# astomodynamics/cddp-cpp

Hardware: AMD Instinct MI355X
Metric: trajectories_per_sec (higher is better)
Workload: dtype f64

## Files before the change

cddp-cpp_amd/csrc/capi.hip:

```cpp
#include <algorithm>
#include <chrono>
#include <cmath>
#include <cstdarg>
#include <cstddef>
#include <cstdio>
#include <cstdlib>
#include <cstring>
#include <string>
#include <vector>
#include <map>

#include "launch.hpp"
#include "plant.hpp"
#include "io_kernels.hpp"
#include "sens_kernels.hpp"
#include "score_kernels.hpp"
#include "mppi_kernels.hpp"

static int ladder_strictly_decreasing(const double *a, int n) {
  for (int i = 1; i < n; ++i) if (!(a[i] < a[i - 1])) return 0;
  return n > 0 ? 1 : 0;
}

using namespace cddp_dev;
// ... 153 lines not shown
  bool initialized = false;
  bool has_state = false;
  bool initial_dirty = false;
  bool ms_cache_started = false;
  size_t bytes = 0;
  int timing_detail = CDDP_HIP_TIMING_ROLLOUT;
  std::vector<hipEvent_t> ev_pool;
  hipEvent_t ev_begin = nullptr, ev_end = nullptr, ev_poll = nullptr, ev_poll2 = nullptr;
  double *d_head = nullptr, *h_head = nullptr; size_t head_cap = 0;
  int *h_poll = nullptr;
  std::map<unsigned long long, hipGraphExec_t> graphs;
  bool shadow_bufs = false;
  int cs_epoch = 0;
  unsigned long long *h_ls = nullptr;
  long long ls_counts[3] = {0, 0, 0};
  int n_redo = 0;
  bool last_shadow = false;
  bool ever_solved = false;
  int *h_bad = nullptr;
  bool has_plan = false;
  double *d_xnext = nullptr;
  double *d_log_u = nullptr, *d_log_x = nullptr; int32_t *d_log_it = nullptr, *d_log_st = nullptr; int log_steps = 0;
};

namespace {

template <class T>
int dalloc(Inner *h, T **p, size_t n) {
  if (n == 0) n = 1;
  void *q = nullptr;
// ... 424 lines not shown
    DA(d.STt, (size_t)d.n_alphas * 8 * Bp); DA(d.YTt, (size_t)d.n_alphas * 8 * Bp); DA(d.GTt, (size_t)d.n_alphas * 8 * Bp);
    DA(d.LamTt, (size_t)d.n_alphas * 16 * Bp);
    if (P.pT > 0) {
      const bool te_coop = h->ks->te_rec_size > 0 && P.mT == 0 && P.pT + 1 <= h->ks->te_group && P.pT <= P.nx;
      const size_t nv = te_coop ? 16 : (size_t)(P.pT + 1);
      DA(d.te_k, nv * N * nu * Bp); DA(d.te_p, nv * (N + 1) * nx * Bp);
      if (te_coop) {
        DA(d.te_cst, (size_t)N * h->ks->te_rec_size * Bp); DA(d.te_cnt, Bp);
        if (!d.dX) DA(d.dX, (size_t)N * nx * Bp);
        if (!d.ys) DA(d.ys, (size_t)N * (m > 0 ? m : 1) * Bp);
      }
    }
  }
  DA(d.n_active, 1);
  DA(d.win_hist, CDDP_HIP_MAX_ALPHAS + 1);
  DA(h->d_launched, ls_words(Bp / 64));
  DA(h->dP, 1);
  DA(h->d_Xinit, d.planeX); DA(h->d_Uinit, d.planeU);
  if (problem->x_ref_traj) {
    DA(h->d_xref_traj, (size_t)(N + 1) * nx);
    hipMemcpyAsync(h->d_xref_traj, problem->x_ref_traj, sizeof(double) * (N + 1) * nx, hipMemcpyHostToDevice, h->stream);
    d.xref_traj = h->d_xref_traj;
  }
#undef DA
  hipMemcpyAsync(h->dP, &h->P, sizeof(ProblemDev), hipMemcpyHostToDevice, h->stream);
  d.P = h->dP;
  d.launched = h->d_launched;
  resolve_route(h);
  if (shadow_layout(h) && knob.costate != Knobs::kCostateSync && !knob.fail_costate && !knob.graph) {
#define DA(ptr, n) do { int rc_ = dalloc(h, &(ptr), (size_t)(n)); if (rc_) { in_destroy(h); return rc_; } } while (0)
    DA(d.Vx2, (size_t)(N + 1) * nx * Bp); DA(d.Vxx2, (size_t)(N + 1) * nx * nx * Bp);
// ... 278 lines not shown
  return 0;
}

struct SolveRun {
  Inner *h = nullptr;
  bool want_stats = false;
  int conc = 1;
  int detail = -1;
  std::vector<int> ev_slot;
  size_t ev_used = 0;
  int launches = 0, outer = 0, it = 0, max_it = 0, na = 0;
  bool two_stage_marks = false, first_rule = true, pinned = false, one_stage = true, done = false, cpu_time_hit = false, use_graph = false;
  int k1 = 1, k_cap = 1, k_cap2 = 1;
  bool shadow = false, force_sync = false, pre_has_state = false, redo_needed = false;
  bool inkernel = false;
  int poll_us = kLsPollUs;
  int stamp0 = 0;
  long waves_all = 0, per_alpha_waves = 1, two_stage_max_waves = 768;
  std::vector<int> hist_now, hist_prev;
  static constexpr int kPollWords = CDDP_HIP_MAX_ALPHAS + 2;
  hipEvent_t poll_evs[2] = {nullptr, nullptr};
  int win_enq = 0, win_dig = 0, win_it[2] = {0, 0};
  int outstanding() const { return win_enq - win_dig; }
  bool ran_ahead = false;
  int post_poll(hipStream_t s) {
    const int slot = win_enq & 1;
    HIPCHK(hipMemcpyAsync(h->h_poll + slot * kPollWords, h->d.n_active, sizeof(int), hipMemcpyDeviceToHost, s));
    HIPCHK(hipMemcpyAsync(h->h_poll + slot * kPollWords + 1, h->d.win_hist, sizeof(int) * (na + 1), hipMemcpyDeviceToHost, s));
    HIPCHK(hipEventRecord(poll_evs[slot], s));
    win_it[slot] = it;
    ++win_enq;
    return 0;
  }
  std::chrono::steady_clock::time_point wall0;
  hipEvent_t fwd_wait = nullptr, fwd_done = nullptr;

  void mark(int point) {
    if (detail < 0) return;
    const bool want = detail == CDDP_HIP_TIMING_ALL ||
                      (detail == CDDP_HIP_TIMING_ROLLOUT && (point == 1 || point == 2 || (two_stage_marks && (point == 3 || point == 4)))) ||
                      (detail == CDDP_HIP_TIMING_SWEEP && (point == 0 || point == 1));
    if (!want) return;
    if (ev_used == h->ev_pool.size()) {
      hipEvent_t e;
      if ((h->knob->event_fence ? hipEventCreate(&e) : hipEventCreateWithFlags(&e, hipEventDisableSystemFence)) != hipSuccess) return;
      h->ev_pool.push_back(e);
    }
    const size_t slot = (size_t)6 * (size_t)(outer - 1) + (size_t)point;
    if (ev_slot.size() <= slot) ev_slot.resize(slot + 1, -1);
    hipEventRecord(h->ev_pool[ev_used], h->stream);
    ev_slot[slot] = (int)ev_used++;
  }

  void adapt_ladder(int window_iters) {
    if (pinned) return;
    long total = 0;
    std::vector<long> hd(na + 1);
    for (int a = 0; a <= na; ++a) { hd[a] = (long)hist_now[a] - (long)hist_prev[a]; total += hd[a]; }
    hist_prev = hist_now;
    if (total <= 0) return;
    const long allow = std::max(1L, (long)window_iters / 4);
    int kq = na;
    long tail = hd[na];
    for (int k = na - 1; k >= 1; --k) {
      tail += hd[k];
      if (tail <= allow) kq = k; else break;
    }
    if (kq >= na - 1) {
      if (waves_all <= 2048) { one_stage = true; }
      else { one_stage = false; k1 = k_cap2; }
    } else {
      one_stage = false; k1 = std::max(1, std::min(kq + h->knob->ls_margin, k_cap));
      if (waves_all <= 2048 && (long)k1 * per_alpha_waves > two_stage_max_waves) one_stage = true;
      const long small_cap = (h->P.solver == CDDP_HIP_SOLVER_LOGDDP || h->P.solver == CDDP_HIP_SOLVER_MSIPDDP) ? 2048 : 1024;
      if (waves_all <= small_cap && h->P.nx <= 8 && h->knob->ls_small_frac * k1 > na) one_stage = true;
    }
    if (h->knob->debug_ladder) {
      std::fprintf(stderr, "[ladder] it=%d total=%ld kq=%d -> %s k1=%d hist:", outer, total, kq, one_stage ? "one" : "two", k1);
      for (int a = 0; a <= na; ++a) std::fprintf(stderr, " %ld", hd[a]);
      std::fprintf(stderr, "\n");
    }
  }

  int begin(Inner *h_, bool stats_, int conc_) {
    h = h_; want_stats = stats_; conc = std::max(1, conc_);
    const ProblemDev &P = h->P;
    const DevBuf &d = h->d;
    hipStream_t s = h->stream;
    const KernelSet *ks = h->ks;
    max_it = P.opt.max_iterations;
    first_rule = (P.ls_rule == CDDP_HIP_LS_FIRST_SUCCESS);
    na = d.n_alphas;
    use_graph = h->knob->graph;
    if (use_graph && conc > 1) {
// ... 3 lines not shown
    detail = (want_stats && !use_graph) ? h->timing_detail : -1;
    if (!h->ev_begin) { HIPCHK(hipEventCreate(&h->ev_begin)); HIPCHK(hipEventCreate(&h->ev_end)); }
    if (!h->ev_poll) { HIPCHK(hipEventCreateWithFlags(&h->ev_poll, hipEventDisableTiming)); HIPCHK(hipEventCreateWithFlags(&h->ev_poll2, hipEventDisableTiming)); }
    poll_evs[0] = h->ev_poll; poll_evs[1] = h->ev_poll2;
    win_enq = win_dig = 0; ran_ahead = false;
    if (!h->h_poll) HIPCHK(hipHostMalloc((void **)&h->h_poll, sizeof(int) * 2 * kPollWords));
    HIPCHK(hipMemsetAsync(h->d_launched, 0, sizeof(unsigned long long) * kLsGran, s));
    HIPCHK(hipEventRecord(h->ev_begin, s));
    pre_has_state = h->has_state;
    shadow = !force_sync && shadow_eligible(h, conc) && max_it > 0;
    redo_needed = false;
    inkernel = shadow && P.ls_rule == CDDP_HIP_LS_FIRST_SUCCESS && h->knob->ls_inkernel &&
               (h->route.rollout == Route::kPair || h->route.rollout == Route::kTwoConsumers);
    poll_us = h->knob->ls_poll_us >= 0 ? h->knob->ls_poll_us : kLsPollUs;
    h->ls_counts[0] = h->ls_counts[1] = h->ls_counts[2] = 0;
    if (inkernel && !h->h_ls) HIPCHK(hipHostMalloc((void **)&h->h_ls, sizeof(unsigned long long) * kLsGran));
    h->last_shadow = shadow; h->ever_solved = true;
    if (shadow) HIPCHK(hipMemsetAsync(h->d.cs_bad, 0, sizeof(int), s));
    stamp0 = h->cs_epoch;
    { int rc = run_initialize(h); if (rc) return rc; }
    launches = 1; outer = 0; it = 0; done = false;
    *h->h_poll = d.B;
    waves_all = (long)conc * (long)((d.B + 63) / 64) * na * (((P.solver == CDDP_HIP_SOLVER_IPDDP && (ks->cst_size > 0 || (d.te_cst && P.m > 0))) || P.solver == CDDP_HIP_SOLVER_MSIPDDP || P.solver == CDDP_HIP_SOLVER_LOGDDP) ? 2 : 1);
    const bool force_two = h->knob->ls_stages == '2', force_one = h->knob->ls_stages == '1';
    const long per_alpha = std::max(1L, waves_all / std::max(1, na));
    per_alpha_waves = per_alpha;
    two_stage_max_waves = h->knob->ls_two_max_waves;
    k_cap = (int)std::max(1L, std::min((long)na - 1, 1024 / per_alpha));
    k_cap2 = (int)std::max(1L, std::min((long)na - 1, 2048 / per_alpha));
    const int k_forced = h->knob->ls_first;
    pinned = !first_rule || na == 1 || force_one || force_two || (k_forced >= 1 && k_forced < na);
    one_stage = !first_rule || na == 1 || force_one || (waves_all <= 2048 && !force_two);
    k1 = force_two ? 1 : k_cap2;
    if (k_forced >= 1 && k_forced < na && !force_one && first_rule) { one_stage = false; k1 = k_forced; }
    hist_now.assign(na + 1, 0); hist_prev.assign(na + 1, 0);
    HIPCHK(hipMemsetAsync(d.win_hist, 0, sizeof(int) * (CDDP_HIP_MAX_ALPHAS + 1), s));
    wall0 = std::chrono::steady_clock::now();
    if (max_it <= 0) { ks->update(d, h->route, 2, 0, 1, 1, s); ++launches; done = true; }
    return 0;
  }

  void enqueue_iteration(int last) {
    const ProblemDev &P = h->P;
    if (shadow) {
      DevBuf &hd = h->d;
      hd.Vx_prev = hd.Vx; hd.Vxx_prev = hd.Vxx;
      std::swap(hd.Vx, hd.Vx2); std::swap(hd.Vxx, hd.Vxx2);
      hd.cs_vsel ^= 1;
    }
    DevBuf dsh = h->d;
    if (shadow) {
      h->cs_epoch += 2;
      dsh.cs_mode = 1; dsh.cs_stamp = h->cs_epoch + 1; dsh.cs_want = dsh.cs_stamp - 2;
      dsh.cs_fail_stamp = h->knob->fail_shadow > 0 ? stamp0 + 2 * h->knob->fail_shadow + 1 : 0;
    }
    const DevBuf &d = dsh;
    hipStream_t s = h->stream;
    const KernelSet *ks = h->ks;
    const Route &r = h->route;
    hipStream_t sf = h->cu.fwd ? h->cu.fwd : s;
    auto to_fwd = [&](int k) { if (sf != s) { order_check(hipEventRecord(h->cu.ev[k], s)); order_check(hipStreamWaitEvent(sf, h->cu.ev[k], 0)); } };
    auto from_fwd = [&](int k) { if (sf != s) { order_check(hipEventRecord(h->cu.ev[k], sf)); order_check(hipStreamWaitEvent(s, h->cu.ev[k], 0)); } };
    const bool split = !one_stage && inkernel;
    two_stage_marks = !one_stage && !split;
    mark(0);
    ks->derivs(d, r, 0, s);
    tl_sweep_hop = h->cu.sweep ? &h->cu.hop : nullptr;
    if (shadow && outer > 1) { dsh.cs_extra = ks->shadow_extra(d, r); ks->backward(dsh, r, P.solver, 0, 1, s); dsh.cs_extra = 0; }
    else ks->backward(d, r, P.solver, 0, 1, s);
    tl_sweep_hop = nullptr;
    mark(1);
    to_fwd(0);
    if (fwd_wait) hipStreamWaitEvent(sf, fwd_wait, 0);
    if (one_stage || split) {
      ks->forward(d, r, P.solver, 0, na, PH_FWD1, 0, first_rule ? 1 : 0, sf, split ? k1 : 0, poll_us);
      if (fwd_done) hipEventRecord(fwd_done, sf);
      from_fwd(1);
      mark(2);
      if (!shadow) ks->costate(d, r, P.solver, 0, na, PH_FWD1, 0, first_rule ? 1 : 2, s);
      ks->update(d, r, 1, na, last, 1, s);
      mark(3);
      launches += shadow ? 3 : 4;
    } else {
      ks->forward(d, r, P.solver, 0, k1, PH_FWD1, 0, 1, sf, 0, 0);
      from_fwd(1);
      mark(2);
      if (!shadow) ks->costate(d, r, P.solver, 0, k1, PH_FWD1, 0, 1, s);
      if (shadow) {
        DevBuf d1 = dsh;
        d1.cs_stamp = h->cs_epoch;
        ks->update(d1, r, 1, k1, last, 0, s);
        d1.cs_want = d1.cs_stamp; d1.Vx_prev = d1.Vx; d1.Vxx_prev = d1.Vxx;
        ks->shadow_flush(d1, nullptr, s);
      } else
      ks->update(d, r, 1, k1, last, 0, s);
      mark(3);
      to_fwd(2);
      ks->forward(d, r, P.solver, k1, na - k1, PH_FWD2, 0, 1, sf, 0, 0);
      if (fwd_done) hipEventRecord(fwd_done, sf);
      from_fwd(3);
      mark(4);
      if (!shadow) ks->costate(d, r, P.solver, k1, na - k1, PH_FWD2, 0, 1, s);
      ks->update(d, r, 2, na, last, 1, s);
      mark(5);
      launches += shadow ? 5 : 6;
    }
  }
  bool polled_iteration(int i) const { return i % h->knob->poll_every == 0 || i == max_it || (i <= 2 && !pinned); }

  int advance_graph() {
    const hipStream_t s = h->stream;
    int w = 0;
    while (it + w < max_it) { ++w; if (polled_iteration(it + w)) break; }
    if (w == 0) { done = true; return 0; }
    const int last = (it + w == max_it) ? 1 : 0;
    const unsigned long long key = ((unsigned long long)(one_stage ? 0 : k1) << 16) | ((unsigned long long)w << 4) | (unsigned long long)last;
    auto f = h->graphs.find(key);
    if (f == h->graphs.end()) {
      hipGraph_t g = nullptr; hipGraphExec_t ge = nullptr;
      const int launches0 = launches;
      HIPCHK(hipStreamBeginCapture(s, hipStreamCaptureModeThreadLocal));
      for (int j = 1; j <= w; ++j) enqueue_iteration((j == w) ? last : 0);
      HIPCHK(hipStreamEndCapture(s, &g));
// ... 62 lines not shown
      df.cs_mode = 1; df.cs_want = h->cs_epoch > stamp0 ? h->cs_epoch + 1 : 0; df.Vx_prev = df.Vx; df.Vxx_prev = df.Vxx;
      df.cs_fail_stamp = h->knob->fail_shadow > 0 ? stamp0 + 2 * h->knob->fail_shadow + 1 : 0;
      h->ks->shadow_flush(df, &dm, s);
      launches += df.cs_want > 0 ? 2 : 1;
      HIPCHK(hipMemsetD32Async((hipDeviceptr_t)d.cs_vbuf, d.cs_vsel, (size_t)d.Bp, s));
      HIPCHK(hipMemcpyAsync(h->h_bad, d.cs_bad, sizeof(int), hipMemcpyDeviceToHost, s));
    }
    return 0;
  }

  int finish(cddp_hip_stats *stats) {
    const DevBuf &d = h->d;
    hipStream_t s = h->stream;
    HIPCHK(hipEventRecord(h->ev_end, s));
    if (inkernel) HIPCHK(hipMemcpyAsync(h->h_ls, h->d_launched, sizeof(unsigned long long) * kLsGran, hipMemcpyDeviceToHost, s));
    HIPCHK(hipStreamSynchronize(s));
    HIPCHK(hipGetLastError());
    if (inkernel) { h->ls_counts[0] = (long long)h->h_ls[kLsRan]; h->ls_counts[1] = (long long)h->h_ls[kLsRet]; h->ls_counts[2] = (long long)h->h_ls[kLsGiveUp]; }
    if (shadow && *h->h_bad != 0) { redo_needed = true; return 0; }
    if (tl_order_error != hipSuccess) {
      const hipError_t oe = tl_order_error; tl_order_error = hipSuccess;
      return fail(-10, "stream ordering (event record / wait) failed during the solve: %s", hipGetErrorString(oe));
    }
    if (!stats) return 0;
    std::memset(stats, 0, sizeof(*stats));
    float ms = 0;
    hipEventElapsedTime(&ms, h->ev_begin, h->ev_end);
    stats->solve_ms = ms;
    auto span = [&](size_t it0, int pa, int pb) -> double {
      const size_t ia = it0 * 6 + (size_t)pa, ib = it0 * 6 + (size_t)pb;
      if (ib >= ev_slot.size() || ev_slot[ia] < 0 || ev_slot[ib] < 0) return 0.0;
      float v = 0;
// ... 427 lines not shown
  if (!h) return -1;
  for (Inner *q : h->g) if (!(q->ever_solved ? q->last_shadow : shadow_eligible(q, std::max(1, std::min(h->conc, (int)h->g.size()))))) return 0;
  return 1;
}
int cddp_hip_costate_redos(cddp_hip_handle *h) {
  if (!h) return -1;
  int n = 0;
  for (Inner *q : h->g) n += q->n_redo;
  return n;
}
int cddp_hip_ls_stage_counts(cddp_hip_handle *h, long long *counts) {
  if (!h || !counts) return -1;
  counts[0] = counts[1] = counts[2] = 0;
  for (Inner *q : h->g) for (int i = 0; i < 3; ++i) counts[i] += q->ls_counts[i];
  return 0;
}
int cddp_hip_concurrency(cddp_hip_handle *h) { return h ? std::max(1, std::min(h->conc, (int)h->g.size())) : -1; }

int cddp_hip_set_timing_detail(cddp_hip_handle *h, int detail) {
  if (!h) return fail(-1, "null handle");
  for (Inner *q : h->g) { int rc = in_set_timing_detail(q, detail); if (rc) return rc; }
  return 0;
}

int cddp_hip_set_stream(cddp_hip_handle *h, void *hip_stream) {
  if (!h) return fail(-1, "null handle");
  h->user_stream = (hipStream_t)hip_stream; h->have_user_stream = true;
  if (h->g.size() == 1) return in_set_stream(h->g[0], hip_stream);
  return 0;
}
// ... 987 lines not shown
```

cddp-cpp_amd/csrc/dev_types.hpp:

```cpp
#pragma once
#include <stdint.h>
#include <stddef.h>
#include "../../include/cddp_hip.h"

namespace cddp_dev {

constexpr int kMaxCons = 4;
constexpr int kMaxTerms = 2;
constexpr int kPool = 1024;
constexpr int kFilterCap = 8;
constexpr int kHistCols = 9;

enum Phase : int { PH_ACTIVE = 0, PH_FWD1 = 1, PH_FWD2 = 2, PH_DONE = 3 };

struct ConDev {
  int kind, dim, dual_dim, offset;
  int off_lower, off_upper, off_center, off_A, off_b;
  int _pad;
  double scale, radius;
};

struct TermDev {
  int kind, dim, offset;
  int off_target, off_A, off_b;
// ... 9 lines not shown
  ConDev cons[kMaxCons];
  TermDev terms[kMaxTerms];
  int off_Qdt, off_Rdt, off_Qf, off_xref;
  double alphas[CDDP_HIP_MAX_ALPHAS];
  double pool[kPool];
};

constexpr int kLS = 64;

constexpr int kSinkDoubles = 1024 * 64;

constexpr int kLsRan = 1, kLsRet = 2, kLsGiveUp = 3, kLsGran = 8;
constexpr unsigned kLsTag = 0x4c533231u;
constexpr size_t ls_words(int NB) { return (size_t)kLsGran + (size_t)NB * CDDP_HIP_MAX_ALPHAS * 2; }
constexpr int kLsPollUs = 10000;

struct DevBuf {
  int B, Bp, N, n_slots, n_alphas, hist_batch, hist_cap, NB;
  int fail_costate_mask;
  const ProblemDev *P;
  const double *xref_traj;
  double *X, *U, *S, *Y, *G, *Lam;
  size_t planeX, planeU, planeM;
  double *A, *Bm, *K, *k, *Vx, *Vxx, *ks, *ky, *Ks, *Ky;
  double *ST, *YT, *GT, *dST, *dYT, *LamT, *dLamT;
  double *STt, *YTt, *GTt, *LamTt;
  double *te_k, *te_p;
  double *te_cst;
  int *te_cnt;
  double *cost, *merit, *inf_pr, *inf_du, *inf_comp, *step_norm, *alpha_pr, *alpha_du, *reg, *mu;
// ... 49 lines not shown
```

cddp-cpp_amd/csrc/kernels.hpp:

```cpp
#pragma once
#include "dev_constraints.hpp"
#include "dev_boxqp.hpp"
#include "dev_models.hpp"
#include "dev_terminal.hpp"

namespace cddp_dev {

#define GI(t, E, e) (((((size_t)(t)) * (size_t)d.NB + (size_t)(b >> 6)) * (E) + (e)) * 64 + (size_t)(b & 63))
#define PIPELINE_FENCE() asm volatile("" ::: "memory")
#define RING_FENCE() asm volatile("s_waitcnt lgkmcnt(0)" ::: "memory")
#define GT(t, E, e) (d.t4 ? ((((size_t)(t) * (size_t)d.NB * 16 + (size_t)(b >> 2)) * (size_t)(E) + (size_t)(e)) * 4 + (size_t)(b & 3)) : GI(t, E, e))
#define G4(t, E, e) ((((size_t)(t) * (size_t)d.NB * 16 + (size_t)(b >> 2)) * (size_t)(E) + (size_t)(e)) * 4 + (size_t)(b & 3))
#define TSTRIDE (d.t4 ? (size_t)4 : (size_t)kLS)

constexpr double kSlackInteriorOffset = 1e-4;
constexpr double kEpsSlack = 1e-10;
constexpr double kMaxBarrierRatio = 1e6;

DEV double clip_pos(double num, double den) { return dclamp(num / den, 0.0, kMaxBarrierRatio); }
DEV double clip_sgn(double num, double den) { return dclamp(num / den, -kMaxBarrierRatio, kMaxBarrierRatio); }

template <int N> DEV void ld(const double *base, size_t stride, double *out) {
#pragma unroll
  for (int i = 0; i < N; ++i) out[i] = base[(size_t)i * stride];
// ... 1453 lines not shown
  const size_t ti = (size_t)a * d.Bp + b;
  const int slot = (a < cur) ? a : a + 1;
  const double a_pr = d.t_apr[ti];
  if ((d.fail_costate_mask >> a) & 1) return false;
  for (int t = 0; t <= d.N; ++t) {
    double xo[NX], lo[NX], vx[NX], xn[NX], lam[NX], vt[NX * (NX + 1) / 2];
    ld<NX>(d.X + (size_t)cur * d.planeX + GI(t, NX, 0), kLS, xo);
    ld<NX>(d.Lam + (size_t)cur * d.planeX + GI(t, NX, 0), kLS, lo);
    ld<NX>(d.Vx + GI(t, NX, 0), kLS, vx);
    ld<NX>(d.X + (size_t)slot * d.planeX + GI(t, NX, 0), kLS, xn);
    costate_load_triangle<NX>(d.Vxx + GI(t, NX * NX, 0), vt);
    if (!costate_row_eval<NX>(lo, vx, vt, xo, xn, a_pr, lam)) return false;
    st<NX>(d.Lam + (size_t)slot * d.planeX + GI(t, NX, 0), kLS, lam);
  }
  return true;
}

template <class Model, class Cons, bool TERM = false>
__global__ __launch_bounds__(64) void k_update(DevBuf d, const ProblemDev *__restrict__ Pk, const double *__restrict__ xrt, int stage, int n1, int is_last_iter, int do_count) {
  constexpr int M = Cons::M;
  constexpr int NXu = Model::NX;
  constexpr int kRB = (NXu <= 6 && !TERM) ? 32 : 16;
  const int b = blockIdx.x * 64 + threadIdx.x;
  if (b >= d.B) return;
  const ProblemDev *__restrict__ P = Pk;
  const cddp_hip_options &o = P->opt;
  const bool ipddp = (P->solver == CDDP_HIP_SOLVER_IPDDP);
  const int ph = d.phase[b];
  const int n_alphas = d.n_alphas;
  int ladder_bin = -1;
// ... 236 lines not shown
            const bool acc = o.acceptable_tolerance > 0.0 && d.inf_pr[b] < at && sdu < at && (nobar || d.inf_comp[b] < at);
            if (acc) st = CDDP_HIP_STATUS_ACCEPTABLE;
          }
          d.status[b] = st; d.phase[b] = PH_DONE;
        } else d.phase[b] = PH_ACTIVE;
      }
    }
  }
count:
  if (d.win_hist) {
    for (int a = 0; a <= n_alphas; ++a) {
      const unsigned long long m = __ballot(ladder_bin == a);
      if (m != 0ull && (int)(threadIdx.x & 63) == __ffsll((long long)m) - 1) atomicAdd(d.win_hist + a, (int)__popcll(m));
    }
  }
  if (do_count) {
    if (is_last_iter && d.phase[b] != PH_DONE) { d.status[b] = CDDP_HIP_STATUS_MAX_ITERATIONS; d.phase[b] = PH_DONE; }
    if (d.phase[b] != PH_DONE) atomicAdd(d.n_active, 1);
  }
}

enum { kInitCold = 0, kInitWarmProvided = 1, kInitWarmExisting = 2 };

DEV void repair_interior(const cddp_hip_options &o, double *s, double *y, int dim) {
  if (!o.ipddp_warmstart_repair) return;
  double mn = INFINITY, mny = INFINITY;
  for (int i = 0; i < dim; ++i) { s[i] = dmax(s[i], o.ipddp_warmstart_s_min); mn = dmin(mn, s[i]); }
  if (mn < o.ipddp_warmstart_s_min * o.ipddp_warmstart_interior_factor) for (int i = 0; i < dim; ++i) s[i] *= o.ipddp_warmstart_interior_factor;
  for (int i = 0; i < dim; ++i) { y[i] = dmax(y[i], o.ipddp_warmstart_y_min); mny = dmin(mny, y[i]); }
  if (mny < o.ipddp_warmstart_y_min * o.ipddp_warmstart_interior_factor) for (int i = 0; i < dim; ++i) y[i] *= o.ipddp_warmstart_interior_factor;
}
DEV bool needs_reinit(const cddp_hip_options &o, const double *y, const double *s, const double *g, int dim) {
  for (int i = 0; i < dim; ++i) if (!dfinite(y[i]) || !dfinite(s[i])) return true;
  for (int i = 0; i < dim; ++i) {
// ... 229 lines not shown
```

cddp-cpp_amd/csrc/kernels_lean.hpp:

```cpp
#pragma once
#include "kernels.hpp"

namespace cddp_dev {

#define GI(t, E, e) (((((size_t)(t)) * (size_t)d.NB + (size_t)(b >> 6)) * (E) + (e)) * 64 + (size_t)(b & 63))

template <class Model, class Cons>
struct CstLayout {
  static constexpr int NX = Model::NX, NU = Model::NU;
  static constexpr int CX = 0, CU = CX + NX, WQYU = CU + NU, QYUSIR = WQYU + NU * NU, IPR = QYUSIR + NU, ICOMP = IPR + 1;
  static constexpr int WQYX = ICOMP + 1, QYXSIR = WQYX + NU * NX, WXQYX = QYXSIR + NX;
  static constexpr int SIZE = Cons::HAS_X ? (WXQYX + NX * NX) : WQYX;
};

template <class Model, class Cons, bool WITH_DERIVS>
DEV void condense_eval(const ProblemDev *__restrict__ P, const double *__restrict__ xrt, const int t, const double *x, const double *u,
                       const double *y, const double *s, const double *g, const double mu, double *A, double *Bq, double *c,
                       double *ys_out = nullptr) {
  constexpr int NX = Model::NX, NU = Model::NU, M = Cons::M;
  typedef Objective<NX, NU> Obj;
  typedef CstLayout<Model, Cons> L;
  const double s_floor = dmax(mu * 1e-3, kEpsSlack);
  double Qyx[M * NX], Qyu[M * NU];
  if constexpr (WITH_DERIVS) {
// ... 600 lines not shown
#else
#define K4_TIME_BEGIN
#define K4_TIME_END(role, steps)
#endif
template <int NX, int NU> struct RollIn { double x[NX], u[NU]; };
template <int NX> struct RollOut { double xn[NX]; };
template <class Model>
__device__ __attribute__((noinline)) RollOut<Model::NX> roll_step_checked(int integrator, double dt, const double *mp, RollIn<Model::NX, Model::NU> in) {
  RollOut<Model::NX> o;
  Stepper<Model>::step(integrator, dt, mp, in.x, in.u, o.xn);
  return o;
}

template <class Model, class Cons, bool TERM = false, int NC = 1>
__global__ __launch_bounds__(64 * (1 + NC)) void k_forward_ipddp_pc(DevBuf d, const ProblemDev *__restrict__ Pk, const double *__restrict__ xrt,
                                                                    int a0, int phase_req, int force, int k1, int poll_us) {
  constexpr int NX = Model::NX, NU = Model::NU, M = Cons::M;
  typedef Objective<NX, NU> Obj;
  static_assert(M > 0, "two-role rollout is for path-constrained problems");
  constexpr int RW = 2 * NX + NU;
  constexpr int kRing = RW <= 10 ? 8 : (RW <= 20 ? 4 : 2);
  __shared__ double s_ring[kRing * RW * 64];
  static_assert(NC == 1 || NC == 2, "one or two consumer waves");
  __shared__ int s_prod;
  __shared__ int s_consv[2];
  [[maybe_unused]] __shared__ int s_abort;
  [[maybe_unused]] __shared__ int s_done1;
  constexpr int kL2 = NC > 1 ? 64 : 1;
  [[maybe_unused]] __shared__ int s_pfail[kL2], s_palive[kL2];
  [[maybe_unused]] __shared__ double s_pmax[4 * kL2];
  [[maybe_unused]] __shared__ double s_prun[kL2];
// ... 614 lines not shown
```

cddp-cpp_amd/csrc/knobs.hpp:

```cpp
#pragma once
#include <climits>
#include <cstdlib>
#include <cstring>
#include <string>

namespace cddp_dev {

inline char env_first(const char *name) { const char *e = std::getenv(name); return e ? e[0] : 0; }
inline bool env_is(const char *name, const char *v) { const char *e = std::getenv(name); return e && !std::strcmp(e, v); }
inline int env_num(const char *name, int dflt, int lo, int hi) { const char *e = std::getenv(name); const int n = e ? std::atoi(e) : dflt; return (n >= lo && n <= hi) ? n : dflt; }
inline long env_long(const char *name, long dflt) { const char *e = std::getenv(name); return e ? std::atol(e) : dflt; }
inline std::string env_str(const char *name) { const char *e = std::getenv(name); return e ? e : ""; }

struct Knobs {
  enum Sweep { kSweepCoop, kSweepLane, kSweepElem, kSweepMfma };
  int sweep = env_is("CDDP_HIP_SWEEP", "lane") ? kSweepLane : env_is("CDDP_HIP_SWEEP", "elem") ? kSweepElem : env_is("CDDP_HIP_SWEEP", "mfma") ? kSweepMfma : kSweepCoop;
  bool t4 = env_first("CDDP_HIP_T4") != '0';
  int sweep_roles = env_num("CDDP_HIP_SWEEP_ROLES", 1, 0, 2);
  bool coop_h2 = env_first("CDDP_HIP_COOP_H") == '2';
  bool coop_w1 = env_first("CDDP_HIP_COOP_W") == '1';
  int k4_na = env_num("CDDP_HIP_K4_NA", 1, 1, 3);
  bool k4_consumers2 = env_first("CDDP_HIP_K4_CONSUMERS") == '2';
  bool ms_lane_rollout = env_is("CDDP_HIP_MS_ROLLOUT", "lane");
  bool lg_lane_rollout = env_is("CDDP_HIP_LG_ROLLOUT", "lane");
  bool graph = env_first("CDDP_HIP_GRAPH") == '1';
  char ls_stages = env_first("CDDP_HIP_LS_STAGES");
  int ls_first = env_num("CDDP_HIP_LS_FIRST", 0, INT_MIN, INT_MAX);
  long ls_two_max_waves = env_long("CDDP_HIP_LS_TWO_MAX_WAVES", 768);
  int ls_small_frac = env_num("CDDP_HIP_LS_SMALL_FRAC", 3, 1, INT_MAX);
  int ls_margin = env_num("CDDP_HIP_LS_MARGIN", 1, 0, 8);
  bool ls_inkernel = env_first("CDDP_HIP_LS_INKERNEL") != '0';
  int ls_poll_us = env_num("CDDP_HIP_TEST_LS_POLL_US", -1, 0, INT_MAX);
  int run_ahead = env_num("CDDP_HIP_RUNAHEAD", 1, 0, 16);
  int poll_every = env_num("CDDP_HIP_POLL_EVERY", 4, 1, INT_MAX);
  bool event_fence = env_first("CDDP_HIP_EVENT_FENCE") == '1';
  bool debug_ladder = std::getenv("CDDP_HIP_DEBUG_LADDER") != nullptr;
  int groups = env_num("CDDP_HIP_GROUPS", 0, INT_MIN, INT_MAX);
  bool chunking = env_num("CDDP_HIP_CHUNK", 1, INT_MIN, INT_MAX) > 0;
  int chunk = env_num("CDDP_HIP_CHUNK", 0, 1, INT_MAX);
  int partition = env_num("CDDP_HIP_PARTITION", 0, 1, 16);
  bool cumask_set = std::getenv("CDDP_HIP_CUMASK") != nullptr;
  std::string cumask = env_str("CDDP_HIP_CUMASK");
  bool pingpong = env_first("CDDP_HIP_PINGPONG") == '1';
  bool xcd_map = env_first("CDDP_HIP_XCD_MAP") != '0';
  int fail_costate = env_num("CDDP_HIP_TEST_FAIL_COSTATE", 0, INT_MIN, INT_MAX);
// ... 7 lines not shown
```

cddp-cpp_amd/host/cddp_hip.hpp:

```cpp
#pragma once
#include <cmath>
#include <cstdlib>
#include <cstring>
#include <exception>
#include <algorithm>
#include <functional>
#include <limits>
#include <iostream>
#include <map>
#include <memory>
#include <stdexcept>
#include <string>
#include <typeinfo>
#include <vector>

#include "../../include/cddp_hip.h"

namespace cddp {

using Vector = std::vector<double>;
struct Matrix {
  int rows = 0, cols = 0;
  std::vector<double> a;
  Matrix() {}
// ... 803 lines not shown
  }
  void mppiBlend(int flags, const cddp_hip_mppi_desc &desc, const double *U_mean, const double *U_cand, const double *cost, const double *viol,
                 double *U_out , double *stats = nullptr) {
    if (!h_) throw std::runtime_error("cddp_hip: mppiBlend needs a resident batch (the plug-in route has no resident handle)");
    check(cddp_hip_mppi_blend(h_, flags, &desc, U_mean, U_cand, cost, viol, U_out, stats));
  }
  void mppiRefine(Plant *plant, int flags, const cddp_hip_mppi_desc &desc, const double *x0 , const double *U_mean ,
                  double *U_out , double *cost_out = nullptr, double *viol_out = nullptr, double *stats = nullptr) {
    if (!h_) throw std::runtime_error("cddp_hip: mppiRefine needs a resident batch (the plug-in route has no resident handle)");
    check(cddp_hip_mppi_refine(h_, plant ? plant->get() : nullptr, flags, &desc, x0, U_mean, U_out, cost_out, viol_out, stats));
  }
  std::vector<CDDPSolution> resolveBatch(CDDP &ctx) {
    if (!h_) throw std::runtime_error("cddp_hip: resolveBatch needs a resident batch (the plug-in route has no resident handle)");
    return collect(ctx, batch_);
  }
  int batch() const { return batch_; }
  cddp_hip_handle *handle() const { return h_; }
  cddp_hip_stats stats{};
  enum class Route { Auto, Plugin, Resident };
  Route route = defaultRoute();
  static Route defaultRoute() {
    const char *e = std::getenv("CDDP_HIP_F4_ROUTE");
    if (e && std::string(e) == "plugin") return Route::Plugin;
    if (e && std::string(e) == "resident") return Route::Resident;
    return Route::Auto;
  }

  static void check(int rc) { if (rc != 0) throw std::runtime_error(std::string("cddp_hip: ") + cddp_hip_last_error()); }

 private:
// ... 305 lines not shown
```

cddp-cpp_amd/pyapi.py:

```python
import ctypes as C
import os
import numpy as np

_HERE = os.path.dirname(os.path.abspath(__file__))
REPO = os.path.dirname(_HERE)
HIP_LIB_PATH = os.environ.get("CDDP_HIP_LIB") or os.path.join(_HERE, "lib", "libcddp_hip.so")

ABI_VERSION = 5
MAX_MODEL_PARAMS = 24
NAME_LEN = 48

MODEL_PENDULUM, MODEL_CARTPOLE, MODEL_UNICYCLE, MODEL_LTI = 0, 1, 2, 3
MODEL_QUADROTOR, MODEL_MANIPULATOR, MODEL_QUADROTOR_EULER12, MODEL_MANIPULATOR7 = 4, 5, 6, 7
MODEL_BICYCLE, MODEL_CAR, MODEL_HCW = 8, 9, 10
MODEL_EULER_ATTITUDE, MODEL_QUATERNION_ATTITUDE, MODEL_MRP_ATTITUDE = 11, 12, 13
MODEL_SPACECRAFT_TWOBODY, MODEL_SPACECRAFT_LANDING2D = 14, 15
MODEL_DUBINS_CAR, MODEL_DREYFUS_ROCKET, MODEL_ACROBOT, MODEL_USV_3DOF, MODEL_FORKLIFT = 16, 17, 18, 19, 20
MODEL_QUADROTOR_RATE, MODEL_SPACECRAFT_LINEAR_FUEL, MODEL_SPACECRAFT_NONLINEAR = 21, 22, 23
EULER, HEUN, RK3, RK4 = 0, 1, 2, 3
SOLVER_CLDDP, SOLVER_IPDDP, SOLVER_LOGDDP, SOLVER_MSIPDDP = 0, 1, 2, 3
CON_CONTROL_BOX, CON_STATE_BOX, CON_BALL, CON_LINEAR = 0, 1, 2, 3
CON_SOC, CON_THRUST, CON_MAX_THRUST = 4, 5, 6
TERM_EQUALITY, TERM_INEQUALITY = 0, 1
STATUS_RUNNING, STATUS_OPTIMAL, STATUS_ACCEPTABLE, STATUS_MAX_ITERATIONS, STATUS_REG_LIMIT, STATUS_MAX_CPU_TIME, STATUS_REG_LIMIT_CONVERGED = range(7)
# ... 727 lines not shown
    "cddp_hip_mppi_blend": [C.c_void_p, C.c_int, C.c_void_p, C.c_void_p, C.c_void_p, C.c_void_p, C.c_void_p, C.c_void_p, C.c_void_p],
    "cddp_hip_mppi_refine": [C.c_void_p, C.c_void_p, C.c_int, C.c_void_p, C.c_void_p, C.c_void_p, C.c_void_p, C.c_void_p, C.c_void_p, C.c_void_p],
}

EXPORTED_SYMBOLS = [
    "cddp_hip_default_options", "cddp_hip_abi_version", "cddp_hip_trig_shared", "cddp_hip_last_error", "cddp_hip_device_count",
    "cddp_hip_status_string", "cddp_hip_build_alphas", "cddp_hip_create", "cddp_hip_destroy",
    "cddp_hip_set_stream", "cddp_hip_set_initial", "cddp_hip_initialize", "cddp_hip_backward",
    "cddp_hip_forward", "cddp_hip_solve", "cddp_hip_get_results", "cddp_hip_get_trajectory",
    "cddp_hip_get_gains", "cddp_hip_get_value", "cddp_hip_get_linearization", "cddp_hip_get_duals", "cddp_hip_get_costates", "cddp_hip_get_backward_scalars",
    "cddp_hip_get_history", "cddp_hip_get_terminal", "cddp_hip_write_gather_records_device", "cddp_hip_dual_dim", "cddp_hip_batch",
    "cddp_hip_set_timing_detail", "cddp_hip_history_capacity", "cddp_hip_set_barrier_state", "cddp_hip_num_groups", "cddp_hip_concurrency", "cddp_hip_comm_unique_id", "cddp_hip_comm_init", "cddp_hip_comm_destroy", "cddp_hip_comm_info", "cddp_hip_get_plan_head", "cddp_hip_allgather_results",
    "cddp_hip_backward_stacks", "cddp_hip_stacks_create_abi", "cddp_hip_stacks_destroy", "cddp_hip_set_stacks", "cddp_hip_set_defect_stack", "cddp_hip_set_control_box", "cddp_hip_set_hessian_stacks", "cddp_hip_set_constraint_stacks",
    "cddp_hip_stacks_backward", "cddp_hip_stacks_last_kernel_ms", "cddp_hip_stacks_last_sweep_form", "cddp_hip_stacks_factor_cache", "cddp_hip_stacks_get_gains", "cddp_hip_stacks_get_constraint_gains",
    "cddp_hip_stacks_get_scalars", "cddp_hip_set_terminal_equality", "cddp_hip_stacks_get_terminal", "cddp_hip_plugin_solve", "cddp_hip_plugin_solve_terminal", "cddp_hip_plugin_set_host_threads", "cddp_hip_plugin_last_stats", "cddp_hip_model_eval", "cddp_hip_set_options", "cddp_hip_set_initial_state", "cddp_hip_forget_solver_state", "cddp_hip_set_duals", "cddp_hip_set_terminal",
    "cddp_hip_costate_mode", "cddp_hip_costate_redos", "cddp_hip_ls_stage_counts", "cddp_hip_mpc_advance", "cddp_hip_mpc_run",
    "cddp_hip_plant_create", "cddp_hip_plant_destroy", "cddp_hip_plant_step", "cddp_hip_mpc_run_plant", "cddp_hip_track_plan",
    "cddp_hip_field_shape", "cddp_hip_get_field_device", "cddp_hip_get_results_device", "cddp_hip_set_initial_device", "cddp_hip_get_live_slots",
    "cddp_hip_plan_jvp", "cddp_hip_plan_vjp",
    "cddp_hip_score_rollouts", "cddp_hip_seed_best",
    "cddp_hip_sample_controls", "cddp_hip_mppi_blend", "cddp_hip_mppi_refine",
]


class HipError(RuntimeError):
    pass


class HipBatchSolver:

    def __init__(self, problem, batch, device=0, trig=None):
# ... 27 lines not shown
        return int(self.lib.cddp_hip_concurrency(self.h))

    def costate_mode(self):
        return int(self.lib.cddp_hip_costate_mode(self.h))

    def costate_redos(self):
        return int(self.lib.cddp_hip_costate_redos(self.h))

    def ls_stage_counts(self):
        c = (C.c_longlong * 3)()
        self.lib.cddp_hip_ls_stage_counts.argtypes = [C.c_void_p, C.POINTER(C.c_longlong)]
        rc = self.lib.cddp_hip_ls_stage_counts(self.h, c)
        if rc != 0:
            raise HipError("cddp_hip_ls_stage_counts failed: %d" % rc)
        return int(c[0]), int(c[1]), int(c[2])

    def set_stream(self, stream_ptr):
        self._check(self.lib.cddp_hip_set_stream(self.h, C.c_void_p(stream_ptr)))
        self._user_stream = True

    def set_timing_detail(self, detail):
        self._check(self.lib.cddp_hip_set_timing_detail(self.h, int(detail)))

    def set_initial(self, x0, U0=None, X0=None):
        x0 = _arr(x0); assert x0.shape == (self.B, self.p.nx)
        U0 = _arr(U0) if U0 is not None else None; X0 = _arr(X0) if X0 is not None else None
        self._check(self.lib.cddp_hip_set_initial(self.h, _ptr(x0), _ptr(U0), _ptr(X0)))

    def initialize(self):
        self.plan_epoch += 1
# ... 892 lines not shown
```

include/cddp_hip.h:

```cpp
#ifndef CDDP_HIP_H
#define CDDP_HIP_H

#include <stdint.h>

#ifdef __cplusplus
extern "C" {
#endif

#define CDDP_HIP_ABI_VERSION 5
#define CDDP_HIP_MAX_MODEL_PARAMS 24
#define CDDP_HIP_NAME_LEN 48
#define CDDP_HIP_MAX_ALPHAS 32


enum cddp_hip_model {
  CDDP_HIP_MODEL_PENDULUM = 0,
  CDDP_HIP_MODEL_CARTPOLE = 1,
  CDDP_HIP_MODEL_UNICYCLE = 2,
  CDDP_HIP_MODEL_LTI = 3,
  CDDP_HIP_MODEL_QUADROTOR = 4,
  CDDP_HIP_MODEL_MANIPULATOR = 5,
  CDDP_HIP_MODEL_QUADROTOR_EULER12 = 6,
  CDDP_HIP_MODEL_MANIPULATOR7 = 7,
  CDDP_HIP_MODEL_BICYCLE = 8,
// ... 249 lines not shown
int cddp_hip_forget_solver_state(cddp_hip_handle *h);

int cddp_hip_set_duals(cddp_hip_handle *h, const double *S, const double *Y);
int cddp_hip_set_terminal(cddp_hip_handle *h, const double *S_T, const double *Y_T, const double *Lambda_T);
int cddp_hip_set_barrier_state(cddp_hip_handle *h, const double *mu, const double *reg);

int cddp_hip_backward(cddp_hip_handle *h, int32_t *ok);

int cddp_hip_forward(cddp_hip_handle *h, const double *alphas, int n_alphas,
                     cddp_hip_trial *trials);

int cddp_hip_solve(cddp_hip_handle *h, cddp_hip_stats *stats);
int cddp_hip_costate_mode(cddp_hip_handle *h);
int cddp_hip_costate_redos(cddp_hip_handle *h);
int cddp_hip_ls_stage_counts(cddp_hip_handle *h, long long *counts);

enum cddp_hip_mpc_mode {
  CDDP_HIP_MPC_KEEP_PLAN = 0,
  CDDP_HIP_MPC_SHIFT_EXISTING = 1,
  CDDP_HIP_MPC_SHIFT_PROVIDED = 2
};
enum { CDDP_HIP_MPC_SHIFT_DUALS = 1,
       CDDP_HIP_MPC_X_DEVICE   = 2 };
int cddp_hip_mpc_advance(cddp_hip_handle *h, int mode, int flags, const double *x_next );
int cddp_hip_mpc_run(cddp_hip_handle *h, int steps, int mode, int flags,
                     double *U_applied , double *X_visited ,
                     int32_t *iterations , int32_t *status , cddp_hip_stats *stats_sum);

typedef struct cddp_hip_plant_desc {
  int32_t abi_version;
// ... 192 lines not shown
```

Before: 110,600.

## Move line-search ladder stage choice onto device with optional in-kernel rule

Factors the two-stage line-search ladder rule into a shared host/device function. Adds an opt-in mode where the last block of the update kernel picks the first-stage alpha count from the window histogram and the forward kernel reads it from device memory. This avoids host histogram copies and polling in early iterations. Also lowers the default ladder margin to zero when the in-kernel line search is active, adds a k1 trace API, and adds a device-side ticket/atomic protocol whose correctness depends on grid-wide ordering.

```diff
diff --git a/cddp-cpp_amd/csrc/capi.hip b/cddp-cpp_amd/csrc/capi.hip
--- a/cddp-cpp_amd/csrc/capi.hip
+++ b/cddp-cpp_amd/csrc/capi.hip
@@ -191,6 +191,8 @@
   int cs_epoch = 0;
   unsigned long long *h_ls = nullptr;
   long long ls_counts[3] = {0, 0, 0};
+  cddp_ladder::Shape ls_shape{};
+  std::vector<int> k1_trace;
   int n_redo = 0;
   bool last_shadow = false;
   bool ever_solved = false;
@@ -645,7 +647,7 @@
   }
   DA(d.n_active, 1);
   DA(d.win_hist, CDDP_HIP_MAX_ALPHAS + 1);
-  DA(h->d_launched, ls_words(Bp / 64));
+  DA(h->d_launched, ls_words(Bp / 64) + kLdWords);
   DA(h->dP, 1);
   DA(h->d_Xinit, d.planeX); DA(h->d_Uinit, d.planeU);
   if (problem->x_ref_traj) {
@@ -954,6 +956,7 @@
   int k1 = 1, k_cap = 1, k_cap2 = 1;
   bool shadow = false, force_sync = false, pre_has_state = false, redo_needed = false;
   bool inkernel = false;
+  bool device_rule = false;
   int poll_us = kLsPollUs;
   int stamp0 = 0;
   long waves_all = 0, per_alpha_waves = 1, two_stage_max_waves = 768;
@@ -966,7 +969,7 @@
   int post_poll(hipStream_t s) {
     const int slot = win_enq & 1;
     HIPCHK(hipMemcpyAsync(h->h_poll + slot * kPollWords, h->d.n_active, sizeof(int), hipMemcpyDeviceToHost, s));
-    HIPCHK(hipMemcpyAsync(h->h_poll + slot * kPollWords + 1, h->d.win_hist, sizeof(int) * (na + 1), hipMemcpyDeviceToHost, s));
+    if (!device_rule) HIPCHK(hipMemcpyAsync(h->h_poll + slot * kPollWords + 1, h->d.win_hist, sizeof(int) * (na + 1), hipMemcpyDeviceToHost, s));
     HIPCHK(hipEventRecord(poll_evs[slot], s));
     win_it[slot] = it;
     ++win_enq;
@@ -993,31 +996,18 @@
   }
 
   void adapt_ladder(int window_iters) {
-    if (pinned) return;
-    long total = 0;
-    std::vector<long> hd(na + 1);
-    for (int a = 0; a <= na; ++a) { hd[a] = (long)hist_now[a] - (long)hist_prev[a]; total += hd[a]; }
+    if (pinned || device_rule) return;
+    std::vector<long long> hd(na + 1);
+    for (int a = 0; a <= na; ++a) hd[a] = (long long)hist_now[a] - (long long)hist_prev[a];
     hist_prev = hist_now;
-    if (total <= 0) return;
-    const long allow = std::max(1L, (long)window_iters / 4);
-    int kq = na;
-    long tail = hd[na];
-    for (int k = na - 1; k >= 1; --k) {
-      tail += hd[k];
-      if (tail <= allow) kq = k; else break;
-    }
-    if (kq >= na - 1) {
-      if (waves_all <= 2048) { one_stage = true; }
-      else { one_stage = false; k1 = k_cap2; }
-    } else {
-      one_stage = false; k1 = std::max(1, std::min(kq + h->knob->ls_margin, k_cap));
-      if (waves_all <= 2048 && (long)k1 * per_alpha_waves > two_stage_max_waves) one_stage = true;
-      const long small_cap = (h->P.solver == CDDP_HIP_SOLVER_LOGDDP || h->P.solver == CDDP_HIP_SOLVER_MSIPDDP) ? 2048 : 1024;
-      if (waves_all <= small_cap && h->P.nx <= 8 && h->knob->ls_small_frac * k1 > na) one_stage = true;
-    }
+    const long long allow = std::max(1LL, (long long)window_iters / 4);
+    const long long *hp = hd.data();
+    const int r = cddp_ladder::first_stage([hp](int a) { return hp[a]; }, h->ls_shape, allow, one_stage ? 0 : k1);
+    one_stage = r == 0;
+    if (r > 0) k1 = r;
     if (h->knob->debug_ladder) {
-      std::fprintf(stderr, "[ladder] it=%d total=%ld kq=%d -> %s k1=%d hist:", outer, total, kq, one_stage ? "one" : "two", k1);
-      for (int a = 0; a <= na; ++a) std::fprintf(stderr, " %ld", hd[a]);
+      std::fprintf(stderr, "[ladder] it=%d -> %s k1=%d hist:", outer, one_stage ? "one" : "two", k1);
+      for (int a = 0; a <= na; ++a) std::fprintf(stderr, " %lld", hd[a]);
       std::fprintf(stderr, "\n");
     }
   }
@@ -1051,7 +1041,7 @@
                (h->route.rollout == Route::kPair || h->route.rollout == Route::kTwoConsumers);
     poll_us = h->knob->ls_poll_us >= 0 ? h->knob->ls_poll_us : kLsPollUs;
     h->ls_counts[0] = h->ls_counts[1] = h->ls_counts[2] = 0;
-    if (inkernel && !h->h_ls) HIPCHK(hipHostMalloc((void **)&h->h_ls, sizeof(unsigned long long) * kLsGran));
+    if (inkernel && !h->h_ls) HIPCHK(hipHostMalloc((void **)&h->h_ls, sizeof(unsigned long long) * kLsGran + sizeof(int) * kLdTraceCap));
     h->last_shadow = shadow; h->ever_solved = true;
     if (shadow) HIPCHK(hipMemsetAsync(h->d.cs_bad, 0, sizeof(int), s));
     stamp0 = h->cs_epoch;
@@ -1072,6 +1062,20 @@
     if (k_forced >= 1 && k_forced < na && !force_one && first_rule) { one_stage = false; k1 = k_forced; }
     hist_now.assign(na + 1, 0); hist_prev.assign(na + 1, 0);
     HIPCHK(hipMemsetAsync(d.win_hist, 0, sizeof(int) * (CDDP_HIP_MAX_ALPHAS + 1), s));
+    device_rule = inkernel && !pinned && !use_graph && h->knob->ls_device;
+    {
+      cddp_ladder::Shape &sh = h->ls_shape;
+      sh.waves_all = waves_all; sh.per_alpha_waves = per_alpha_waves; sh.two_stage_max_waves = two_stage_max_waves;
+      sh.na = na; sh.k_cap = k_cap; sh.k_cap2 = k_cap2; sh.nx = P.nx;
+      sh.two_role_small = (P.solver == CDDP_HIP_SOLVER_LOGDDP || P.solver == CDDP_HIP_SOLVER_MSIPDDP) ? 1 : 0;
+      sh.small_frac = h->knob->ls_small_frac; sh.whole_slack = h->knob->ls_whole_slack;
+      sh.margin = h->knob->ls_margin >= 0 ? h->knob->ls_margin : (inkernel ? 0 : 1);
+    }
+    h->k1_trace.clear();
+    if (device_rule) {
+      HIPCHK(hipMemcpyAsync(h->d_launched + ls_words(d.NB), &h->ls_shape, sizeof(h->ls_shape), hipMemcpyHostToDevice, s));
+      if (!one_stage) HIPCHK(hipMemsetD32Async((hipDeviceptr_t)((int *)(h->d_launched + kLdWord) + kLdK1), k1, 1, s));
+    }
     wall0 = std::chrono::steady_clock::now();
     if (max_it <= 0) { ks->update(d, h->route, 2, 0, 1, 1, s); ++launches; done = true; }
     return 0;
@@ -1098,8 +1102,9 @@
     hipStream_t sf = h->cu.fwd ? h->cu.fwd : s;
     auto to_fwd = [&](int k) { if (sf != s) { order_check(hipEventRecord(h->cu.ev[k], s)); order_check(hipStreamWaitEvent(sf, h->cu.ev[k], 0)); } };
     auto from_fwd = [&](int k) { if (sf != s) { order_check(hipEventRecord(h->cu.ev[k], sf)); order_check(hipStreamWaitEvent(s, h->cu.ev[k], 0)); } };
-    const bool split = !one_stage && inkernel;
+    const bool split = (!one_stage || device_rule) && inkernel;
     two_stage_marks = !one_stage && !split;
+    if (!device_rule) h->k1_trace.push_back(one_stage ? 0 : k1);
     mark(0);
     ks->derivs(d, r, 0, s);
     tl_sweep_hop = h->cu.sweep ? &h->cu.hop : nullptr;
@@ -1110,12 +1115,12 @@
     to_fwd(0);
     if (fwd_wait) hipStreamWaitEvent(sf, fwd_wait, 0);
     if (one_stage || split) {
-      ks->forward(d, r, P.solver, 0, na, PH_FWD1, 0, first_rule ? 1 : 0, sf, split ? k1 : 0, poll_us);
+      ks->forward(d, r, P.solver, 0, na, PH_FWD1, 0, first_rule ? 1 : 0, sf, device_rule ? -1 : (split ? k1 : 0), poll_us);
       if (fwd_done) hipEventRecord(fwd_done, sf);
       from_fwd(1);
       mark(2);
       if (!shadow) ks->costate(d, r, P.solver, 0, na, PH_FWD1, 0, first_rule ? 1 : 2, s);
-      ks->update(d, r, 1, na, last, 1, s);
+      ks->update(d, r, 1, na, last, device_rule ? (1 | 2 | (outer << 2)) : 1, s);
       mark(3);
       launches += shadow ? 3 : 4;
     } else {
@@ -1143,7 +1148,7 @@
       launches += shadow ? 5 : 6;
     }
   }
-  bool polled_iteration(int i) const { return i % h->knob->poll_every == 0 || i == max_it || (i <= 2 && !pinned); }
+  bool polled_iteration(int i) const { return i % h->knob->poll_every == 0 || i == max_it || (i <= 2 && !pinned && !device_rule); }
 
   int advance_graph() {
     const hipStream_t s = h->stream;
@@ -1236,8 +1241,11 @@
     hipStream_t s = h->stream;
     HIPCHK(hipEventRecord(h->ev_end, s));
     if (inkernel) HIPCHK(hipMemcpyAsync(h->h_ls, h->d_launched, sizeof(unsigned long long) * kLsGran, hipMemcpyDeviceToHost, s));
+    const int n_trace = device_rule ? std::min(outer, kLdTraceCap) : 0;
+    if (n_trace > 1) HIPCHK(hipMemcpyAsync(h->h_ls + kLsGran, (const char *)(h->d_launched + ls_words(d.NB)) + offsetof(LadderDev, trace), sizeof(int) * n_trace, hipMemcpyDeviceToHost, s));
     HIPCHK(hipStreamSynchronize(s));
     HIPCHK(hipGetLastError());
+    if (n_trace > 0) { const int *t = (const int *)(h->h_ls + kLsGran); h->k1_trace.assign(t, t + n_trace); h->k1_trace[0] = one_stage ? 0 : k1; }
     if (inkernel) { h->ls_counts[0] = (long long)h->h_ls[kLsRan]; h->ls_counts[1] = (long long)h->h_ls[kLsRet]; h->ls_counts[2] = (long long)h->h_ls[kLsGiveUp]; }
     if (shadow && *h->h_bad != 0) { redo_needed = true; return 0; }
     if (tl_order_error != hipSuccess) {
@@ -1695,6 +1703,12 @@
   counts[0] = counts[1] = counts[2] = 0;
   for (Inner *q : h->g) for (int i = 0; i < 3; ++i) counts[i] += q->ls_counts[i];
   return 0;
+}
+int cddp_hip_ls_k1_trace(cddp_hip_handle *h, int *k1, int cap) {
+  if (!h || h->g.empty() || cap < 0 || (cap > 0 && !k1)) return -1;
+  const std::vector<int> &t = h->g[0]->k1_trace;
+  for (int i = 0; i < cap && i < (int)t.size(); ++i) k1[i] = t[i];
+  return (int)t.size();
 }
 int cddp_hip_concurrency(cddp_hip_handle *h) { return h ? std::max(1, std::min(h->conc, (int)h->g.size())) : -1; }
 
diff --git a/cddp-cpp_amd/csrc/dev_types.hpp b/cddp-cpp_amd/csrc/dev_types.hpp
--- a/cddp-cpp_amd/csrc/dev_types.hpp
+++ b/cddp-cpp_amd/csrc/dev_types.hpp
@@ -2,6 +2,7 @@
 #include <stdint.h>
 #include <stddef.h>
 #include "../../include/cddp_hip.h"
+#include "ladder_rule.hpp"
 
 namespace cddp_dev {
 
@@ -47,6 +48,16 @@
 constexpr unsigned kLsTag = 0x4c533231u;
 constexpr size_t ls_words(int NB) { return (size_t)kLsGran + (size_t)NB * CDDP_HIP_MAX_ALPHAS * 2; }
 constexpr int kLsPollUs = 10000;
+
+constexpr int kLdWord = 4, kLdTicket = 0, kLdK1 = 1;
+constexpr int kLdWindow = 4;
+constexpr int kLdTraceCap = 1024;
+struct LadderDev {
+  cddp_ladder::Shape shape;
+  int ring[kLdWindow][CDDP_HIP_MAX_ALPHAS + 1];
+  int trace[kLdTraceCap];
+};
+constexpr size_t kLdWords = (sizeof(LadderDev) + 7) / 8;
 
 struct DevBuf {
   int B, Bp, N, n_slots, n_alphas, hist_batch, hist_cap, NB;
diff --git a/cddp-cpp_amd/csrc/kernels.hpp b/cddp-cpp_amd/csrc/kernels.hpp
--- a/cddp-cpp_amd/csrc/kernels.hpp
+++ b/cddp-cpp_amd/csrc/kernels.hpp
@@ -1491,6 +1491,31 @@
     st<NX>(d.Lam + (size_t)slot * d.planeX + GI(t, NX, 0), kLS, lam);
   }
   return true;
+}
+
+DEV void ladder_choose(const DevBuf &d, int it) {
+  __shared__ int s_hd[CDDP_HIP_MAX_ALPHAS + 1];
+  int *const w = (int *)(d.launched + kLdWord);
+  LadderDev *const L = (LadderDev *)(d.launched + ls_words(d.NB));
+  const cddp_ladder::Shape sh = L->shape;
+  asm volatile("s_waitcnt vmcnt(0)" ::: "memory");
+  if (__hip_atomic_fetch_add(w + kLdTicket, 1, __ATOMIC_RELAXED, __HIP_MEMORY_SCOPE_AGENT) != (int)gridDim.x - 1) return;
+  __hip_atomic_store(w + kLdTicket, 0, __ATOMIC_RELAXED, __HIP_MEMORY_SCOPE_AGENT);
+  const int na = d.n_alphas;
+  int *const row = L->ring[it % kLdWindow];
+  const int keep = __hip_atomic_load(w + kLdK1, __ATOMIC_RELAXED, __HIP_MEMORY_SCOPE_AGENT);
+  int now[CDDP_HIP_MAX_ALPHAS + 1], old[CDDP_HIP_MAX_ALPHAS + 1];
+#pragma unroll
+  for (int a = 0; a <= CDDP_HIP_MAX_ALPHAS; ++a) {
+    now[a] = (a <= na) ? __hip_atomic_fetch_add(d.win_hist + a, 0, __ATOMIC_RELAXED, __HIP_MEMORY_SCOPE_AGENT) : 0;
+    old[a] = (a <= na && it > kLdWindow) ? row[a] : 0;
+  }
+#pragma unroll
+  for (int a = 0; a <= CDDP_HIP_MAX_ALPHAS; ++a)
+    if (a <= na) { s_hd[a] = now[a] - old[a]; row[a] = now[a]; }
+  const int k1 = cddp_ladder::first_stage([&](int a) { return (long long)s_hd[a]; }, sh, 1, keep);
+  __hip_atomic_store(w + kLdK1, k1, __ATOMIC_RELAXED, __HIP_MEMORY_SCOPE_AGENT);
+  if (it < kLdTraceCap) L->trace[it] = k1;
 }
 
 template <class Model, class Cons, bool TERM = false>
@@ -1757,10 +1782,11 @@
       if (m != 0ull && (int)(threadIdx.x & 63) == __ffsll((long long)m) - 1) atomicAdd(d.win_hist + a, (int)__popcll(m));
     }
   }
-  if (do_count) {
+  if (do_count & 1) {
     if (is_last_iter && d.phase[b] != PH_DONE) { d.status[b] = CDDP_HIP_STATUS_MAX_ITERATIONS; d.phase[b] = PH_DONE; }
     if (d.phase[b] != PH_DONE) atomicAdd(d.n_active, 1);
   }
+  if ((do_count & 2) && threadIdx.x == 0) ladder_choose(d, do_count >> 2);
 }
 
 enum { kInitCold = 0, kInitWarmProvided = 1, kInitWarmExisting = 2 };
diff --git a/cddp-cpp_amd/csrc/kernels_lean.hpp b/cddp-cpp_amd/csrc/kernels_lean.hpp
--- a/cddp-cpp_amd/csrc/kernels_lean.hpp
+++ b/cddp-cpp_amd/csrc/kernels_lean.hpp
@@ -638,7 +638,8 @@
 
 template <class Model, class Cons, bool TERM = false, int NC = 1>
 __global__ __launch_bounds__(64 * (1 + NC)) void k_forward_ipddp_pc(DevBuf d, const ProblemDev *__restrict__ Pk, const double *__restrict__ xrt,
-                                                                    int a0, int phase_req, int force, int k1, int poll_us) {
+                                                                    int a0, int phase_req, int force, int k1_arg, int poll_us) {
+  const int k1 = k1_arg >= 0 ? k1_arg : __builtin_amdgcn_readfirstlane(((const int *)(d.launched + kLdWord))[kLdK1]);
   constexpr int NX = Model::NX, NU = Model::NU, M = Cons::M;
   typedef Objective<NX, NU> Obj;
   static_assert(M > 0, "two-role rollout is for path-constrained problems");
diff --git a/cddp-cpp_amd/csrc/knobs.hpp b/cddp-cpp_amd/csrc/knobs.hpp
--- a/cddp-cpp_amd/csrc/knobs.hpp
+++ b/cddp-cpp_amd/csrc/knobs.hpp
@@ -28,7 +28,9 @@
   int ls_first = env_num("CDDP_HIP_LS_FIRST", 0, INT_MIN, INT_MAX);
   long ls_two_max_waves = env_long("CDDP_HIP_LS_TWO_MAX_WAVES", 768);
   int ls_small_frac = env_num("CDDP_HIP_LS_SMALL_FRAC", 3, 1, INT_MAX);
-  int ls_margin = env_num("CDDP_HIP_LS_MARGIN", 1, 0, 8);
+  int ls_margin = env_num("CDDP_HIP_LS_MARGIN", -1, 0, 8);
+  bool ls_device = env_first("CDDP_HIP_LS_DEVICE") == '1';
+  int ls_whole_slack = env_num("CDDP_HIP_LS_WHOLE_SLACK", 1, -1, INT_MAX);
   bool ls_inkernel = env_first("CDDP_HIP_LS_INKERNEL") != '0';
   int ls_poll_us = env_num("CDDP_HIP_TEST_LS_POLL_US", -1, 0, INT_MAX);
   int run_ahead = env_num("CDDP_HIP_RUNAHEAD", 1, 0, 16);
diff --git a/cddp-cpp_amd/csrc/ladder_rule.hpp b/cddp-cpp_amd/csrc/ladder_rule.hpp
--- /dev/null
+++ b/cddp-cpp_amd/csrc/ladder_rule.hpp
@@ -0,0 +1,46 @@
+#pragma once
+
+#if defined(__HIPCC__)
+#define CDDP_LADDER_HD __host__ __device__
+#else
+#define CDDP_LADDER_HD
+#endif
+
+namespace cddp_ladder {
+
+struct Shape {
+  long long waves_all;
+  long long per_alpha_waves;
+  long long two_stage_max_waves;
+  int na;
+  int k_cap, k_cap2;
+  int nx;
+  int two_role_small;
+  int small_frac;
+  int margin;
+  int whole_slack;
+};
+
+template <class Hist>
+CDDP_LADDER_HD inline int first_stage(const Hist &hd, const Shape &s, long long allow, int keep) {
+  const int na = s.na;
+  long long total = 0;
+  for (int a = 0; a <= na; ++a) total += hd(a);
+  if (total <= 0) return keep;
+  int kq = na;
+  long long tail = hd(na);
+  for (int k = na - 1; k >= 1; --k) {
+    tail += hd(k);
+    if (tail <= allow) kq = k; else break;
+  }
+  if (s.whole_slack >= 0 && kq >= na - s.whole_slack) return s.waves_all <= 2048 ? 0 : s.k_cap2;
+  int k1 = kq + s.margin;
+  if (k1 > s.k_cap) k1 = s.k_cap;
+  if (k1 < 1) k1 = 1;
+  if (s.waves_all <= 2048 && (long long)k1 * s.per_alpha_waves > s.two_stage_max_waves) return 0;
+  const long long small_cap = s.two_role_small ? 2048 : 1024;
+  if (s.waves_all <= small_cap && s.nx <= 8 && (long long)s.small_frac * k1 > na) return 0;
+  return k1;
+}
+
+}
diff --git a/cddp-cpp_amd/host/cddp_hip.hpp b/cddp-cpp_amd/host/cddp_hip.hpp
--- a/cddp-cpp_amd/host/cddp_hip.hpp
+++ b/cddp-cpp_amd/host/cddp_hip.hpp
@@ -841,6 +841,14 @@
     if (!h_) throw std::runtime_error("cddp_hip: resolveBatch needs a resident batch (the plug-in route has no resident handle)");
     return collect(ctx, batch_);
   }
+  std::vector<int> lsK1Trace() {
+    if (!h_) throw std::runtime_error("cddp_hip: lsK1Trace needs a resident batch (the plug-in route has no resident handle)");
+    const int n = cddp_hip_ls_k1_trace(h_, nullptr, 0);
+    if (n < 0) throw std::runtime_error("cddp_hip: cddp_hip_ls_k1_trace failed");
+    std::vector<int> k1((size_t)n);
+    if (n > 0) cddp_hip_ls_k1_trace(h_, k1.data(), n);
+    return k1;
+  }
   int batch() const { return batch_; }
   cddp_hip_handle *handle() const { return h_; }
   cddp_hip_stats stats{};
diff --git a/cddp-cpp_amd/pyapi.py b/cddp-cpp_amd/pyapi.py
--- a/cddp-cpp_amd/pyapi.py
+++ b/cddp-cpp_amd/pyapi.py
@@ -765,7 +765,7 @@
     "cddp_hip_backward_stacks", "cddp_hip_stacks_create_abi", "cddp_hip_stacks_destroy", "cddp_hip_set_stacks", "cddp_hip_set_defect_stack", "cddp_hip_set_control_box", "cddp_hip_set_hessian_stacks", "cddp_hip_set_constraint_stacks",
     "cddp_hip_stacks_backward", "cddp_hip_stacks_last_kernel_ms", "cddp_hip_stacks_last_sweep_form", "cddp_hip_stacks_factor_cache", "cddp_hip_stacks_get_gains", "cddp_hip_stacks_get_constraint_gains",
     "cddp_hip_stacks_get_scalars", "cddp_hip_set_terminal_equality", "cddp_hip_stacks_get_terminal", "cddp_hip_plugin_solve", "cddp_hip_plugin_solve_terminal", "cddp_hip_plugin_set_host_threads", "cddp_hip_plugin_last_stats", "cddp_hip_model_eval", "cddp_hip_set_options", "cddp_hip_set_initial_state", "cddp_hip_forget_solver_state", "cddp_hip_set_duals", "cddp_hip_set_terminal",
-    "cddp_hip_costate_mode", "cddp_hip_costate_redos", "cddp_hip_ls_stage_counts", "cddp_hip_mpc_advance", "cddp_hip_mpc_run",
+    "cddp_hip_costate_mode", "cddp_hip_costate_redos", "cddp_hip_ls_stage_counts", "cddp_hip_ls_k1_trace", "cddp_hip_mpc_advance", "cddp_hip_mpc_run",
     "cddp_hip_plant_create", "cddp_hip_plant_destroy", "cddp_hip_plant_step", "cddp_hip_mpc_run_plant", "cddp_hip_track_plan",
     "cddp_hip_field_shape", "cddp_hip_get_field_device", "cddp_hip_get_results_device", "cddp_hip_set_initial_device", "cddp_hip_get_live_slots",
     "cddp_hip_plan_jvp", "cddp_hip_plan_vjp",
@@ -823,6 +823,15 @@
         if rc != 0:
             raise HipError("cddp_hip_ls_stage_counts failed: %d" % rc)
         return int(c[0]), int(c[1]), int(c[2])
+
+    def ls_k1_trace(self):
+        self.lib.cddp_hip_ls_k1_trace.argtypes = [C.c_void_p, C.POINTER(C.c_int), C.c_int]
+        n = self.lib.cddp_hip_ls_k1_trace(self.h, None, 0)
+        if n < 0:
+            raise HipError("cddp_hip_ls_k1_trace failed: %d" % n)
+        k = (C.c_int * max(n, 1))()
+        self.lib.cddp_hip_ls_k1_trace(self.h, k, n)
+        return [int(k[i]) for i in range(n)]
 
     def set_stream(self, stream_ptr):
         self._check(self.lib.cddp_hip_set_stream(self.h, C.c_void_p(stream_ptr)))
diff --git a/include/cddp_hip.h b/include/cddp_hip.h
--- a/include/cddp_hip.h
+++ b/include/cddp_hip.h
@@ -287,6 +287,7 @@
 int cddp_hip_costate_mode(cddp_hip_handle *h);
 int cddp_hip_costate_redos(cddp_hip_handle *h);
 int cddp_hip_ls_stage_counts(cddp_hip_handle *h, long long *counts);
+int cddp_hip_ls_k1_trace(cddp_hip_handle *h, int *k1, int cap);
 
 enum cddp_hip_mpc_mode {
   CDDP_HIP_MPC_KEEP_PLAN = 0,
```

Measured after the change: 112,800 (median of 6 runs). No clear change (+1.9%).
